# ccuchengwei/LongReadSelfCorrect

Hardware: NVIDIA B200
Metric: corrected Mbp/s (seed + FM-extend + DP/MSA fallback, default options) (higher is better)
Workload: dtype int64+f64

## Files before the change

include/pbsc.h:

```cpp
#ifndef PBSC_H
#define PBSC_H

#include <stddef.h>
#include <stdint.h>

#ifdef __cplusplus
extern "C" {
#endif

#define PBSC_OK 0
#define PBSC_ERR_ARG (-1)
#define PBSC_ERR_IO (-2)
#define PBSC_ERR_FORMAT (-3)
#define PBSC_ERR_CUDA (-4)
#define PBSC_ERR_LIMIT (-5)
#define PBSC_ERR_INTERNAL (-6)

#define PBSC_BWT 0
#define PBSC_RBWT 1

#define PBSC_WALK_OK 1
#define PBSC_WALK_HIGH_ERROR (-1)
#define PBSC_WALK_EXCEED_DEPTH (-2)
#define PBSC_WALK_EXCEED_LEAVES (-3)
// ... 110 lines not shown
int pbsc_batch_run(pbsc_batch* b, float* ms);
int pbsc_batch_result_size(pbsc_batch* b, uint64_t* piece_bytes, uint64_t* n_pieces);
int pbsc_batch_fetch(pbsc_batch* b, char* pieces_out, uint64_t pieces_cap, uint64_t* piece_offsets,
                     uint64_t piece_offsets_cap, uint64_t* first_piece, pbsc_read_stats* stats);
void pbsc_batch_destroy(pbsc_batch* b);

typedef struct pbsc_walk_log { int32_t src_start, trg_start, code, dp_failed; } pbsc_walk_log;
int pbsc_batch_debug_size(pbsc_batch* b, uint64_t* n_seeds, uint64_t* n_log);
int pbsc_batch_fetch_debug(pbsc_batch* b, pbsc_seed* seeds, uint64_t seeds_cap, uint64_t* seed_offsets, uint32_t* n_surviving, float* ratio,
                           uint64_t ratio_cap, pbsc_walk_log* log, uint64_t log_cap, uint64_t* log_offsets);

typedef struct pbsc_timing
{
    float h2d_ms, seed_ms, extend_ms, d2h_ms, total_ms;
    uint64_t kernel_launches;
    uint64_t seed_pairs;
    uint64_t rank_queries;
    float dp_ms;
    uint64_t dp_jobs;
    uint64_t dp_rows;
    float walk_ms;
    uint64_t walk_launches;
    uint64_t dp_thread_rows;
} pbsc_timing;
int pbsc_last_timing(pbsc_timing* t);
int pbsc_occ_counts(uint64_t* out, int reset);

#define PBSC_BUILD_NO_FORWARD 1
#define PBSC_BUILD_NO_REVERSE 2
int pbsc_build_index_files(const char* reads, const uint64_t* offsets, uint64_t n_reads, const char* prefix, int device, int flags);
int pbsc_build_bwt(const char* reads, const uint64_t* offsets, uint64_t n_reads, int reverse, int device, uint8_t** runs, uint64_t* n_runs,
                   uint64_t* n_symbols, uint32_t** lex_order);
void pbsc_free(void* p);

#ifdef __cplusplus
}
#endif
#endif
```

longreadselfcorrect_b200/api.py:

```python
from __future__ import annotations

import ctypes as C
import os
from dataclasses import dataclass

import numpy as np

_PKG = os.path.dirname(os.path.abspath(__file__))
LIB_PATH = os.environ.get("PBSC_LIB") or os.path.join(_PKG, "libpbsc.so")

PBSC_BWT, PBSC_RBWT = 0, 1


class PbscError(RuntimeError):
    def __init__(self, code: int, msg: str):
        super().__init__(f"pbsc error {code}: {msg}")
        self.code = code


class CParams(C.Structure):
    _fields_ = [
        ("pb_coverage", C.c_int32), ("error_rate", C.c_double), ("start_kmer", C.c_int32), ("next_target", C.c_int32),
        ("max_leaves", C.c_int32), ("idmer_len", C.c_int32), ("min_kmer", C.c_int32), ("genome", C.c_int32),
        ("mode", C.c_int32), ("manual", C.c_int32), ("adjust", C.c_int32), ("split", C.c_int32), ("no_dp", C.c_int32),
        ("offset", C.c_int32 * 3), ("pool", C.c_int32 * 8), ("n_pool", C.c_int32), ("scan_kmer", C.c_int32),
        ("kmer_up_bound", C.c_int32), ("radius", C.c_int32), ("hh_ratio", C.c_float),
        ("threshold", (C.c_float * 52) * 3), ("freqs_of_kmer", C.c_double * 101),
        ("debug_seed", C.c_int32), ("reserved", C.c_int32),
    ]


class CSeed(C.Structure):
    _fields_ = [("start", C.c_int32), ("len", C.c_int32), ("max_fixed_freq", C.c_int32), ("is_repeat", C.c_int32),
                ("start_best_k", C.c_int32), ("end_best_k", C.c_int32), ("hitchhiked", C.c_int32), ("static_k", C.c_int32)]


class CReadStats(C.Structure):
    _fields_ = [(n, C.c_int64) for n in ("total_reads_len", "corrected_len", "total_seed_num", "total_walk_num",
                                          "high_error_num", "exceed_depth_num", "exceed_leave_num", "fm_num", "dp_num",
                                          "seed_dis")] + [("merge", C.c_int32), ("n_pieces", C.c_int32)]


class CTiming(C.Structure):
    _fields_ = [("h2d_ms", C.c_float), ("seed_ms", C.c_float), ("extend_ms", C.c_float), ("d2h_ms", C.c_float),
                ("total_ms", C.c_float), ("kernel_launches", C.c_uint64), ("seed_pairs", C.c_uint64),
                ("rank_queries", C.c_uint64), ("dp_ms", C.c_float), ("dp_jobs", C.c_uint64), ("dp_rows", C.c_uint64),
                ("walk_ms", C.c_float), ("walk_launches", C.c_uint64), ("dp_thread_rows", C.c_uint64)]


SEED_DTYPE = np.dtype([("start", "<i4"), ("len", "<i4"), ("max_fixed_freq", "<i4"), ("is_repeat", "<i4"),
                       ("start_best_k", "<i4"), ("end_best_k", "<i4"), ("hitchhiked", "<i4"), ("static_k", "<i4")])
STATS_DTYPE = np.dtype([(n, "<i8") for n in ("total_reads_len", "corrected_len", "total_seed_num", "total_walk_num",
                                             "high_error_num", "exceed_depth_num", "exceed_leave_num", "fm_num",
                                             "dp_num", "seed_dis")] + [("merge", "<i4"), ("n_pieces", "<i4")])

WALK_LOG_DTYPE = np.dtype([("src_start", "<i4"), ("trg_start", "<i4"), ("code", "<i4"), ("dp_failed", "<i4")])

EXPORTED = ["pbsc_last_error", "pbsc_device_count", "pbsc_params_default", "pbsc_params_derive",
            "pbsc_threshold_table_text", "pbsc_index_create", "pbsc_index_load", "pbsc_index_create_synthetic",
            "pbsc_index_build_prefix_table", "pbsc_index_destroy", "pbsc_index_num_symbols", "pbsc_index_num_strings",
            "pbsc_index_device_bytes", "pbsc_index_get_symbols", "pbsc_findinterval_batch", "pbsc_findinterval_device",
            "pbsc_seed_batch", "pbsc_extend_batch", "pbsc_correct_batch", "pbsc_last_timing",
            "pbsc_batch_upload", "pbsc_batch_run", "pbsc_batch_result_size", "pbsc_batch_fetch", "pbsc_batch_destroy",
            "pbsc_host_alloc", "pbsc_host_free", "pbsc_trim", "pbsc_random_sector_bench",
            "pbsc_index_save", "pbsc_index_load_fmg", "pbsc_index_open", "pbsc_index_clone", "pbsc_index_blob_size",
            "pbsc_index_export_blob", "pbsc_index_import_blob", "pbsc_index_set_lanes", "pbsc_index_lanes",
            "pbsc_host_register", "pbsc_host_unregister", "pbsc_occ_counts",
            "pbsc_batch_debug_size", "pbsc_batch_fetch_debug",
            "pbsc_build_index_files", "pbsc_build_bwt", "pbsc_free"]

# ... 442 lines not shown
```

longreadselfcorrect_b200/csrc/pbsc_dp.cu:

```cuda
#include <cub/cub.cuh>
#include <stdio.h>
#include <stdlib.h>
#include <string.h>
#include <algorithm>
#include <vector>
#include <type_traits>
#include "pbsc_batch.cuh"
#include "pbsc_task.cuh"
#include <chrono>
#include "pbsc_dp.cuh"
#include "pbsc_dp_thread.cuh"
#include "pbsc_dp_msa.cuh"

namespace pbsc {

constexpr int DP_HALF = 100;
constexpr int DP_BW = 2 * DP_HALF + 1;
constexpr int DP_CPL = 7;
constexpr int DP_NEG = -(1 << 28);
constexpr int DP_WARPS = 8;

struct __align__(16) DpJob
{
    uint64_t lo[4];
// ... 579 lines not shown
__global__ void __launch_bounds__(128)
dp_job_keys_kernel(uint64_t j0, uint64_t j1, const DpJob* __restrict__ jobs, const DpRow* __restrict__ rows, uint64_t row_base, uint32_t* keys,
                   uint32_t* order)
{
    const uint64_t t = blockIdx.x * (uint64_t)blockDim.x + threadIdx.x;
    if (j0 + t >= j1) return;
    const DpJob J = jobs[j0 + t];
    const uint32_t nr = job_rows_of(J);
    const DpRow* R = rows + (J.row0 - row_base);
    uint32_t passing = 0, cost = 0;
    for (uint32_t r = 0; r < nr; r++)
    {
        const DpRow x = R[r];
        if (x.pass == 1) { passing++; cost += x.nops; }
    }
    if (passing < 3) cost = 0;
    keys[t] = 0xFFFFu - min(0xFFFFu, cost >> 3);
    order[t] = (uint32_t)t;
}

__global__ void __launch_bounds__(64)
dp_msa_kernel(uint64_t j0, uint64_t j1, const uint32_t* __restrict__ order, int deal, const DpJob* __restrict__ jobs, WalkTask* tasks,
              const DpRow* __restrict__ rows, uint64_t row_base, uint8_t* mem, uint64_t mem0, uint8_t* outpool, unsigned int* n_bad,
              uint32_t big_thr, uint32_t* big_list, unsigned int* n_big)
{
    const uint64_t tx = blockIdx.x * (uint64_t)blockDim.x + threadIdx.x;
    const uint64_t njc = j1 - j0;
    uint64_t rank = tx;
    if (order && deal)
    {
        const uint64_t n_warps = (njc + 31) / 32;
        rank = (tx & 31) * n_warps + (tx >> 5);
        if (tx >= n_warps * 32) return;
    }
    if (rank >= njc) return;
    const uint64_t jx = j0 + (order ? order[rank] : rank);
    const DpJob J = jobs[jx];
    WalkTask& tk = tasks[J.task];
    const uint32_t nr = job_rows_of(J);
    const DpRow* R = rows + (J.row0 - row_base);
    if (big_list)
    {
        uint32_t cost = 0, passing = 0;
        for (uint32_t r = 0; r < nr; r++) { const DpRow x = R[r]; if (x.pass == 1) { passing++; cost += x.nops; } }
        if (passing >= 3 && cost >= big_thr) { big_list[atomicAdd(n_big, 1u)] = (uint32_t)(jx - j0); return; }
    }
    JobView v;
    job_view(mem + (J.mem - mem0), J, nr, v);
    const MsaCtx ctx{tk, outpool};
    uint32_t n = 0;
    const int rc = msa::consensus(v, J.qlen, J.k, R, nr, ctx, n);
    if (rc == 1) { tk.dp_status = PBSC_DP_FEW_ROWS; return; }
    if (rc == 2) { atomicAdd(n_bad, 1u); tk.dp_status = PBSC_OVF_DP; return; }
    tk.out_len = n;
    tk.dp_status = PBSC_DP_OK;
}

constexpr int MSA_WARPS = 4;
__global__ void __launch_bounds__(MSA_WARPS * 32)
dp_msa_warp_kernel(uint64_t j0, const uint32_t* __restrict__ big_list, const unsigned int* __restrict__ n_big, unsigned long long* counter,
                   const DpJob* __restrict__ jobs, WalkTask* tasks, const DpRow* __restrict__ rows, uint64_t row_base, uint8_t* mem, uint64_t mem0,
                   uint8_t* outpool, unsigned int* n_bad)
{
    __shared__ unsigned int gap_counter[MSA_WARPS];
    const int lane = threadIdx.x & 31, warp = threadIdx.x >> 5;
    const unsigned long long n = *n_big;
    for (;;)
    {
        unsigned long long it = 0;
        if (lane == 0) it = atomicAdd(counter, 1ull);
        it = __shfl_sync(0xffffffffu, it, 0);
        if (it >= n) break;
        const uint64_t jx = j0 + big_list[it];
        const DpJob J = jobs[jx];
        WalkTask& tk = tasks[J.task];
        const uint32_t nr = job_rows_of(J);
        const DpRow* R = rows + (J.row0 - row_base);
        JobView v;
        job_view(mem + (J.mem - mem0), J, nr, v);
        const MsaCtx ctx{tk, outpool};
        uint32_t nout = 0;
        const int rc = msa::consensus_warp(v, J.qlen, J.k, R, nr, ctx, nout, &gap_counter[warp]);
        __syncwarp();
        if (lane == 0)
        {
            if (rc == 1) tk.dp_status = PBSC_DP_FEW_ROWS;
            else if (rc == 2) { atomicAdd(n_bad, 1u); tk.dp_status = PBSC_OVF_DP; }
            else { tk.out_len = nout; tk.dp_status = PBSC_DP_OK; }
        }
        __syncwarp();
    }
}

template <class T>
static cudaError_t arena(pbsc_index* idx, const char* name, size_t count, T** out) { return arena_get(idx, name, (count ? count : 1) * sizeof(T), (void**)out); }

DpStats& last_dp_stats() { static thread_local DpStats s; return s; }

struct DptPass
{
    bool on = false; uint64_t qmax = 0, arena_words = 0, min_rows = 0, read_words = 0; int blocks = 0;
    uint64_t flag_words() const { return on ? arena_words * (uint64_t)blocks : 0; }
};
template <class C>
static cudaError_t dpt_pass_setup(pbsc_index* idx, uint64_t q_longest, uint64_t q_prev_max, int cap_per_sm, DptPass& g)
{
    g.on = q_longest > q_prev_max;
    if (!g.on) return cudaSuccess;
    g.qmax = std::min<uint64_t>((uint64_t)C::QMAX, q_longest);
    g.arena_words = 32ull * g.qmax * dpt::WMAX;
    cudaError_t e = cudaFuncSetAttribute(dp_align_thread_kernel<C>, cudaFuncAttributeMaxDynamicSharedMemorySize, C::SMEM);
    if (e != cudaSuccess) return e;
    int per = 0;
    e = cudaOccupancyMaxActiveBlocksPerMultiprocessor(&per, dp_align_thread_kernel<C>, C::NT, C::SMEM);
// ... 18 lines not shown
}

int run_dp_fallback(pbsc_index* idx, const pbsc_params* p, DeviceBatch& b, void* tasks_v, uint64_t n_items, const uint32_t* list, uint8_t* outpool,
                    uint32_t q_cap, uint64_t* launches)
{
    WalkTask* tasks = (WalkTask*)tasks_v;
    cudaStream_t st = idx->stream;
    if (n_items == 0) return PBSC_OK;
    const bool htrace = getenv("PBSC_ROUND_TRACE") != nullptr;
    auto h0 = std::chrono::steady_clock::now();
    auto hmark = [&](const char* what) {
        if (!htrace) return;
        const auto now = std::chrono::steady_clock::now();
        const double ms = std::chrono::duration<double, std::milli>(now - h0).count();
        if (ms > 2.0) fprintf(stderr, "[pbsc round trace]     dp host: %-22s %8.2f ms\n", what, ms);
        h0 = now;
    };
    DpJob* jobs; uint64_t *job_rows, *job_bytes, *row_off, *mem_off; unsigned int* cnt; unsigned long long* qctr;
    PBSC_CUDA(arena(idx, "dp.jobs", n_items, &jobs));
    PBSC_CUDA(arena(idx, "dp.job_rows", n_items + 1, &job_rows));
    PBSC_CUDA(arena(idx, "dp.job_bytes", n_items + 1, &job_bytes));
    PBSC_CUDA(arena(idx, "dp.row_off", n_items + 1, &row_off));
    PBSC_CUDA(arena(idx, "dp.mem_off", n_items + 1, &mem_off));
    PBSC_CUDA(arena(idx, "dp.cnt", 4, &cnt));
    PBSC_CUDA(arena(idx, "dp.qctr", 4, &qctr));
    PBSC_CUDA(cudaMemsetAsync(cnt, 0, 16, st));
    cudaEvent_t ev[2];
    PBSC_CUDA(cudaEventCreate(&ev[0])); PBSC_CUDA(cudaEventCreate(&ev[1]));
    struct EvGuard { cudaEvent_t* e; ~EvGuard() { cudaEventDestroy(e[0]); cudaEventDestroy(e[1]); } } guard{ev};
    PBSC_CUDA(cudaEventRecord(ev[0], st));
    dp_collect_kernel<<<(unsigned)((n_items + 127) / 128), 128, 0, st>>>(idx->dev, n_items, list, tasks, b.codes.p, b.offsets.p, (uint32_t)p->pb_coverage,
                                                                        jobs, job_rows, job_bytes, cnt);
    unsigned int hcnt[4] = {0, 0, 0, 0};
    PBSC_CUDA(cudaMemcpyAsync(hcnt, cnt, 16, cudaMemcpyDeviceToHost, st));
    PBSC_CUDA(cudaStreamSynchronize(st));
    if (launches) *launches += 1;
    const uint64_t nj = hcnt[0];
    DpStats& S = last_dp_stats();
    hmark("collect + sync");
    if (nj == 0) return PBSC_OK;
    {
        size_t tb = 0, tb2 = 0;
        cub::DeviceScan::ExclusiveSum(nullptr, tb, job_rows, row_off, (int)(nj + 1), st);
        cub::DeviceScan::ExclusiveSum(nullptr, tb2, job_bytes, mem_off, (int)(nj + 1), st);
        tb = std::max(tb, tb2);
        uint8_t* tmp;
        PBSC_CUDA(arena(idx, "dp.cubtmp", tb, &tmp));
        PBSC_CUDA(cudaMemsetAsync(job_rows + nj, 0, 8, st));
        PBSC_CUDA(cudaMemsetAsync(job_bytes + nj, 0, 8, st));
        cub::DeviceScan::ExclusiveSum(tmp, tb, job_rows, row_off, (int)(nj + 1), st);
        cub::DeviceScan::ExclusiveSum(tmp, tb, job_bytes, mem_off, (int)(nj + 1), st);
        dp_offsets_kernel<<<(unsigned)((nj + 255) / 256), 256, 0, st>>>(nj, jobs, row_off, mem_off);
    }
    std::vector<uint64_t> h_row(nj + 1), h_mem(nj + 1);
    PBSC_CUDA(cudaMemcpyAsync(h_row.data(), row_off, (nj + 1) * 8, cudaMemcpyDeviceToHost, st));
    PBSC_CUDA(cudaMemcpyAsync(h_mem.data(), mem_off, (nj + 1) * 8, cudaMemcpyDeviceToHost, st));
// ... 65 lines not shown
        cub::DeviceRadixSort::SortPairs(nullptr, sort_bytes, tkeys, tkeys2, torder, torder2, (int)max_rows, 0, DPT_KEY_BITS, st);
        PBSC_CUDA(arena(idx, "dp.sorttmp", sort_bytes, &sort_tmp));
        PBSC_CUDA(arena(idx, "dp.tflags", std::max(pass_s.flag_words(), std::max(pass_l.flag_words(), pass_h.flag_words())), &tslabs));
        PBSC_CUDA(arena(idx, "dp.treads", std::max<uint64_t>(1, std::max(pass_l.on ? pass_l.read_words : 0, pass_h.on ? pass_h.read_words : 0)), &treads));
    }
    int sort_jobs = 0;
    if (const char* e = getenv("PBSC_DP_SORT_JOBS")) sort_jobs = atoi(e);
    uint32_t *jkeys = nullptr, *jkeys2 = nullptr, *jord = nullptr, *jord2 = nullptr;
    uint8_t* jsort_tmp = nullptr;
    size_t jsort_bytes = 0;
    if (sort_jobs)
    {
        PBSC_CUDA(arena(idx, "dp.jkeys", nj, &jkeys));
        PBSC_CUDA(arena(idx, "dp.jkeys2", nj, &jkeys2));
        PBSC_CUDA(arena(idx, "dp.jord", nj, &jord));
        PBSC_CUDA(arena(idx, "dp.jord2", nj, &jord2));
        cub::DeviceRadixSort::SortPairs(nullptr, jsort_bytes, jkeys, jkeys2, jord, jord2, (int)nj, 0, 16, st);
        PBSC_CUDA(arena(idx, "dp.jsorttmp", jsort_bytes, &jsort_tmp));
    }
    uint32_t msa_big_thr = 8192;
    if (const char* e = getenv("PBSC_MSA_WARP_MIN")) msa_big_thr = atoll(e) < 0 ? 0xffffffffu : (uint32_t)atoll(e);
    uint32_t* msa_big = nullptr;
    unsigned long long* msa_q = nullptr;
    PBSC_CUDA(arena(idx, "dp.msa_big", nj, &msa_big));
    PBSC_CUDA(arena(idx, "dp.msa_q", 2, &msa_q));
    struct Prof
    {
        bool on = false; cudaStream_t st; std::vector<std::pair<const char*, cudaEvent_t>> ev;
        void mark(const char* name) { if (!on) return; cudaEvent_t e; cudaEventCreate(&e); cudaEventRecord(e, st); ev.emplace_back(name, e); }
        void report()
        {
            if (!on || ev.size() < 2) return;
            cudaEventSynchronize(ev.back().second);
            std::vector<std::pair<const char*, float>> acc;
            for (size_t x = 1; x < ev.size(); x++)
            {
                float ms = 0; cudaEventElapsedTime(&ms, ev[x - 1].second, ev[x].second);
                bool found = false;
                for (auto& a : acc) if (!strcmp(a.first, ev[x].first)) { a.second += ms; found = true; }
                if (!found) acc.emplace_back(ev[x].first, ms);
            }
            fprintf(stderr, "[pbsc dp profile]");
            for (auto& a : acc) fprintf(stderr, " %s %.1f ms;", a.first, a.second);
            fprintf(stderr, "\n");
            for (auto& e : ev) cudaEventDestroy(e.second);
        }
    } prof;
    prof.st = st;
    if (const char* e = getenv("PBSC_DP_PROFILE")) prof.on = atoi(e) != 0;
    hmark("pass setup + arenas");
    prof.mark("start");
    for (uint64_t j0 = 0; j0 < nj;)
    {
        uint64_t j1 = j0 + 1;
        while (j1 < nj && h_mem[j1 + 1] - h_mem[j0] <= pool_bytes) j1++;
        const uint64_t nrows = h_row[j1] - h_row[j0], njc = j1 - j0;
        dp_rows_kernel<<<(unsigned)((njc + 127) / 128), 128, 0, st>>>(j0, j1, jobs, tasks, b.codes.p, b.offsets.p, mem, h_mem[j0], rows, h_row[j0]);
        dp_retrieve_kernel<<<(unsigned)((nrows + 127) / 128), 128, 0, st>>>(idx->dev, nrows, rows, jobs, mem, h_mem[j0]);
        prof.mark("rows+retrieve");
        PBSC_CUDA(cudaMemsetAsync(qctr, 0, 32, st));
        if (pass_s.on)
        {
            dpt_pass_launch<DptShort>(pass_s, st, nrows, rows, jobs, tasks, mem, h_mem[j0], tkeys, tkeys2, torder, torder2, sort_tmp, sort_bytes, tslabs,
                                      qctr + 1, cnt, treads);
            prof.mark("align_thread_256");
            if (launches) *launches += 4;
        }
        if (pass_l.on)
        {
            dpt_pass_launch<DptLong>(pass_l, st, nrows, rows, jobs, tasks, mem, h_mem[j0], tkeys, tkeys2, torder, torder2, sort_tmp, sort_bytes, tslabs,
                                     qctr + 1, cnt, treads);
            prof.mark("align_thread_1024");
            if (launches) *launches += 4;
        }
        if (pass_h.on)
        {
            dpt_pass_launch<DptHuge>(pass_h, st, nrows, rows, jobs, tasks, mem, h_mem[j0], tkeys, tkeys2, torder, torder2, sort_tmp, sort_bytes, tslabs,
                                     qctr + 1, cnt, treads);
            prof.mark("align_thread_4000");
            if (launches) *launches += 4;
        }
        const int nb = (int)std::min<uint64_t>((uint64_t)ablocks, (nrows + DP_WARPS * 32 - 1) / (DP_WARPS * 32));
        dp_align_kernel<<<nb, DP_WARPS * 32, 0, st>>>(nrows, rows, jobs, tasks, mem, h_mem[j0], slabs, arena_words, qctr, cnt + 1);
        prof.mark("align_warp");
        const uint32_t* jorder = nullptr;
        if (sort_jobs)
        {
            dp_job_keys_kernel<<<(unsigned)((njc + 127) / 128), 128, 0, st>>>(j0, j1, jobs, rows, h_row[j0], jkeys, jord);
            size_t sb = jsort_bytes;
            cub::DeviceRadixSort::SortPairs(jsort_tmp, sb, jkeys, jkeys2, jord, jord2, (int)njc, 0, 16, st);
            jorder = jord2;
            if (launches) *launches += 3;
        }
        PBSC_CUDA(cudaMemsetAsync(msa_q, 0, 16, st));
        dp_msa_kernel<<<(unsigned)((((njc + 31) / 32) * 32 + 63) / 64), 64, 0, st>>>(j0, j1, jorder, sort_jobs == 1, jobs, tasks, rows, h_row[j0], mem,
                                                                                         h_mem[j0], outpool, cnt + 1, msa_big_thr,
                                                                                         msa_big_thr != 0xffffffffu ? msa_big : nullptr, (unsigned int*)(msa_q + 1));
        prof.mark("msa");
        if (msa_big_thr != 0xffffffffu)
        {
            const int wb = (int)std::min<uint64_t>((uint64_t)idx->sm_count * 4, (njc + MSA_WARPS - 1) / MSA_WARPS);
            dp_msa_warp_kernel<<<wb, MSA_WARPS * 32, 0, st>>>(j0, msa_big, (const unsigned int*)(msa_q + 1), msa_q, jobs, tasks, rows, h_row[j0], mem, h_mem[j0],
                                                              outpool, cnt + 1);
            prof.mark("msa_warp");
            if (launches) *launches += 1;
        }
        PBSC_CUDA(cudaGetLastError());
        if (launches) *launches += 4;
        S.chunks++;
        j0 = j1;
    }
    PBSC_CUDA(cudaEventRecord(ev[1], st));
    hmark("chunk loop (launches)");
    prof.report();
    PBSC_CUDA(cudaMemcpyAsync(hcnt, cnt, 12, cudaMemcpyDeviceToHost, st));
    PBSC_CUDA(cudaStreamSynchronize(st));
    S.bad += hcnt[1];
    S.thread_rows += hcnt[2];
    PBSC_OCC_TAKE(3, st);
    float ms = 0;
    cudaEventElapsedTime(&ms, ev[0], ev[1]);
    S.ms += ms;
    return PBSC_OK;
}

}
```

longreadselfcorrect_b200/csrc/pbsc_dp.cuh:

```cuda
#ifndef PBSC_DP_CUH
#define PBSC_DP_CUH

#include "pbsc_batch.cuh"

namespace pbsc {

struct DpStats { uint64_t jobs = 0, rows = 0, chunks = 0, bad = 0, thread_rows = 0; float ms = 0; };
DpStats& last_dp_stats();

int run_dp_fallback(pbsc_index* idx, const pbsc_params* p, DeviceBatch& b, void* tasks, uint64_t n_items, const uint32_t* list, uint8_t* outpool,
                    uint32_t q_cap, uint64_t* launches);

}
#endif
```

longreadselfcorrect_b200/csrc/pbsc_dp_msa.cuh:

```cuda
#ifndef PBSC_DP_MSA_CUH
#define PBSC_DP_MSA_CUH

#include <stdint.h>

#if defined(__CUDACC__)
#define PBSC_MSA_HD __host__ __device__ __forceinline__
#define PBSC_MSA_ALIGN(n) __align__(n)
#else
#define PBSC_MSA_HD inline
#define PBSC_MSA_ALIGN(n) alignas(n)
#endif

namespace pbsc {

constexpr int OP_M = 0, OP_I = 1, OP_D = 2;

struct PBSC_MSA_ALIGN(16) DpRow
{
    uint32_t job, local;
    uint32_t len, seq_start;
    uint32_t nops;
    int32_t start0, start1;
    uint32_t pass;
};
// ... 94 lines not shown
#endif
        for (int s = 0; s < 5; s++) if ((int)cnt[s] > maxCount) { maxSym = s; maxCount = cnt[s]; }
        const int baseCount = cnt[baseSym];
        return (maxCount >= baseCount && baseCount < minCall) ? maxSym : baseSym;
    };
    bool over = false;
    for (uint32_t p = 0; p < qlen && !over; p++)
    {
        if (p >= 1)
            for (uint32_t g = v.head[p]; g; g = v.pool[g - 1].next)
            {
                const int s = call(v.pool[g - 1].cnt, 4);
                if (s != 4) { if (n >= cap) { over = true; break; } out[n++] = (uint8_t)s; }
            }
        if (over) break;
        const int s = call(v.baseCnt + p * 5, (int)q[p]);
        if (s != 4) { if (n >= cap) { over = true; break; } out[n++] = (uint8_t)s; }
    }
    if (over || n < k) return 2;
    n_out = n;
    return 0;
}

#if defined(__CUDACC__)
template <class Ctx>
__device__ __forceinline__ int consensus_warp(const JobView& v, const uint32_t qlen, const uint32_t k, const DpRow* R, const uint32_t nr, const Ctx& ctx,
                                              uint32_t& n_out, unsigned int* gap_counter)
{
    const unsigned FULLW = 0xffffffffu;
    const int lane = threadIdx.x & 31;
    uint32_t passing = 0;
    for (uint32_t r = lane; r < nr; r += 32) passing += R[r].pass == 1;
    #pragma unroll
    for (int o = 16; o > 0; o >>= 1) passing += __shfl_xor_sync(FULLW, passing, o);
    if (passing < 3) return 1;
    const uint8_t* q = v.q;
    for (uint32_t p = lane; p <= qlen; p += 32)
    {
        #pragma unroll
        for (int c = 0; c < 5; c++) v.baseCnt[p * 5 + c] = 0;
        v.startAt[p] = p == 0 ? 1 : 0; v.head[p] = 0; v.tail[p] = 0;
        if (p < qlen) v.baseCnt[p * 5 + q[p]] = 1;
    }
    if (lane == 0) *gap_counter = 0;
    __syncwarp();
    const uint32_t gapCap = dp_gap_cap(qlen);
    bool bad = false;
    for (uint32_t r = 0; r < nr; r++)
    {
        if (R[r].pass != 1) continue;
        const uint8_t* buf = v.rows + (uint64_t)R[r].local * v.rowBytes;
        const uint8_t* s2 = buf + R[r].seq_start;
        const uint8_t* ops = buf + v.seqBytes;
        const int nops = (int)R[r].nops;
        const int chunk = (nops + 31) / 32;
        int t0 = min(lane * chunk, nops);
        while (t0 > 0 && t0 < nops && ops[nops - t0] == OP_I) t0++;
        int t1 = __shfl_down_sync(FULLW, t0, 1);
        if (lane == 31) t1 = nops;
        uint32_t md = 0, mi = 0;
        for (int t = t0; t < t1; t++) { const int op = ops[nops - 1 - t]; md += op != OP_I; mi += op != OP_D; }
        uint32_t pmd = md, pmi = mi;
        #pragma unroll
        for (int o = 1; o < 32; o <<= 1)
        {
            const uint32_t a = __shfl_up_sync(FULLW, pmd, o), b = __shfl_up_sync(FULLW, pmi, o);
            if (lane >= o) { pmd += a; pmi += b; }
        }
        uint32_t p = (uint32_t)R[r].start0 + (pmd - md), inc = (uint32_t)R[r].start1 + (pmi - mi);
        bool firstOp = t0 == 0;
        uint32_t cur = (t0 == 0 || t0 >= t1) ? 0 : v.head[p];
        int t = t0;
        while (t < t1)
        {
            const int op = ops[nops - 1 - t];
            if (cur)
            {
                GapCol& g = v.pool[cur - 1];
                if (op == OP_I) { g.cnt[s2[inc]]++; inc++; t++; firstOp = false; }
                else g.cnt[4]++;
                cur = g.next;
            }
            else if (op == OP_I)
            {
                const uint32_t slot = atomicAdd(gap_counter, 1u);
                if (slot >= gapCap) { bad = true; break; }
                uint32_t cover = 0;
                #pragma unroll
                for (int s = 0; s < 5; s++) cover += v.baseCnt[p * 5 + s];
                GapCol g;
                g.cnt[0] = g.cnt[1] = g.cnt[2] = g.cnt[3] = 0; g.pad = 0; g.next = 0;
                g.cnt[4] = (uint16_t)(cover - v.startAt[p]);
                g.cnt[s2[inc]] = 1;
                v.pool[slot] = g;
                if (v.tail[p]) v.pool[v.tail[p] - 1].next = slot + 1; else v.head[p] = slot + 1;
                v.tail[p] = slot + 1;
                inc++; t++; firstOp = false;
            }
            else
            {
                if (p >= qlen) { bad = true; break; }
                v.baseCnt[p * 5 + (op == OP_M ? s2[inc] : 4)]++;
                if (op == OP_M) inc++;
                if (firstOp) v.startAt[p]++;
                firstOp = false;
                p++; t++;
                cur = v.head[p];
            }
        }
        __syncwarp();
        if (__any_sync(FULLW, bad)) return 2;
    }
    const int minCall = ctx.min_call();
    uint8_t* out = ctx.out();
    const uint32_t cap = ctx.cap();
    auto call = [&](const uint16_t* cnt, int baseSym) -> int
    {
        int maxSym = -1, maxCount = -1;
        #pragma unroll
        for (int s = 0; s < 5; s++) if ((int)cnt[s] > maxCount) { maxSym = s; maxCount = cnt[s]; }
        const int baseCount = cnt[baseSym];
        return (maxCount >= baseCount && baseCount < minCall) ? maxSym : baseSym;
    };
    const uint32_t blk = (qlen + 31) / 32;
    const uint32_t pa = min((uint32_t)lane * blk, qlen), pb = min(pa + blk, qlen);
    uint32_t n = 0;
    #pragma unroll 1
    for (int pass = 0; pass < 2; pass++)
    {
        uint32_t w = 0;
        if (pass == 1)
        {
            uint32_t incl = n;
            #pragma unroll
            for (int o = 1; o < 32; o <<= 1) { const uint32_t a = __shfl_up_sync(FULLW, incl, o); if (lane >= o) incl += a; }
            const uint32_t total = __shfl_sync(FULLW, incl, 31);
            if (total > cap || total < k) return 2;
            n_out = total;
            w = incl - n;
        }
        for (uint32_t p = pa; p < pb; p++)
        {
            if (p >= 1)
                for (uint32_t g = v.head[p]; g; g = v.pool[g - 1].next)
                {
                    const int s = call(v.pool[g - 1].cnt, 4);
                    if (s != 4) { if (pass == 0) n++; else out[w++] = (uint8_t)s; }
                }
            const int s = call(v.baseCnt + p * 5, (int)q[p]);
            if (s != 4) { if (pass == 0) n++; else out[w++] = (uint8_t)s; }
        }
    }
    return 0;
}
#endif

}
}

#endif
```

longreadselfcorrect_b200/csrc/pbsc_index.cu:

```cuda
#include <math.h>
#include <string.h>
#include <sys/stat.h>
#include <algorithm>
#include <cub/cub.cuh>
#include <mutex>
#include <map>
#include <fstream>
#include <sstream>
#include "pbsc_internal.h"

namespace pbsc {

static thread_local std::string g_err;
void set_error(const char* fmt, ...)
{
    char buf[1024];
    va_list ap;
    va_start(ap, fmt);
    vsnprintf(buf, sizeof buf, fmt, ap);
    va_end(ap);
    g_err = buf;
}
int cuda_fail(cudaError_t e, const char* what, const char* file, int line)
{
// ... 978 lines not shown
}
PBSC_CATCH_ALL("pbsc_threshold_table_text")

int pbsc_occ_counts(uint64_t* out, int reset)
{
    if (!out) return PBSC_ERR_ARG;
    unsigned long long* c = occ_counts();
    for (int i = 0; i < 5; i++) { out[i] = c[i]; if (reset) c[i] = 0; }
#ifdef PBSC_COUNT_OCC
    return 1;
#else
    return 0;
#endif
}

int pbsc_last_timing(pbsc_timing* t)
{
    if (!t) return PBSC_ERR_ARG;
    const Timing& s = last_timing();
    t->h2d_ms = s.h2d_ms; t->seed_ms = s.seed_ms; t->extend_ms = s.extend_ms; t->d2h_ms = s.d2h_ms; t->total_ms = s.total_ms;
    t->kernel_launches = s.kernel_launches; t->seed_pairs = s.seed_pairs; t->rank_queries = s.rank_queries;
    t->dp_ms = s.dp_ms; t->dp_jobs = s.dp_jobs; t->dp_rows = s.dp_rows;
    t->walk_ms = s.walk_ms; t->walk_launches = s.walk_launches; t->dp_thread_rows = s.dp_thread_rows;
    return PBSC_OK;
}

}
```

longreadselfcorrect_b200/csrc/pbsc_internal.h:

```cpp
#ifndef PBSC_INTERNAL_H
#define PBSC_INTERNAL_H

#include <cuda_runtime.h>
#include <stdarg.h>
#include <stdint.h>
#include <stdio.h>
#include <stdlib.h>
#include <chrono>
#include <exception>
#include <map>
#include <new>
#include <mutex>
#include <condition_variable>
#include <string>
#include <vector>
#include "../../include/pbsc.h"
#include "fm_table.cuh"
#include "pbsc_status.h"

struct pbsc_index
{
    int device = 0;
    pbsc::FmIndexDev dev;
    pbsc::FmBlock* d_blocks[2] = {nullptr, nullptr};
// ... 70 lines not shown
        const auto t0 = std::chrono::steady_clock::now();
        if (a.p) cudaFree(a.p);
        a.p = nullptr; a.cap = 0;
        const size_t want = bytes + bytes / 8 + 256;
        cudaError_t e = cudaMalloc(&a.p, want);
        if (e != cudaSuccess) return e;
        a.cap = want;
        if (tr) fprintf(stderr, "[pbsc round trace]     arena %-16s -> %8.1f MB in %7.2f ms\n", name, want / 1048576.0,
                        std::chrono::duration<double, std::milli>(std::chrono::steady_clock::now() - t0).count());
    }
    *out = a.p;
    return cudaSuccess;
}

struct Timing
{
    float h2d_ms = 0, seed_ms = 0, extend_ms = 0, d2h_ms = 0, total_ms = 0;
    uint64_t kernel_launches = 0, seed_pairs = 0, rank_queries = 0;
    float dp_ms = 0;
    uint64_t dp_jobs = 0, dp_rows = 0;
    float walk_ms = 0;
    uint64_t walk_launches = 0;
    uint64_t dp_thread_rows = 0;
};
Timing& last_timing();

#define PBSC_MAX_LANES 4
int lane_acquire(pbsc_index* primary, int idmer_len, pbsc_index** lane);
void lane_release(pbsc_index* primary, pbsc_index* lane);
int ensure_idmer_table(pbsc_index* idx, int idmer_len);

inline int base_code(char b) { switch (b) { case 'A': return 0; case 'C': return 1; case 'G': return 2; case 'T': return 3; default: return -1; } }

}
#endif
```

longreadselfcorrect_b200/csrc/pbsc_pipeline.cu:

```cuda
#include <string.h>
#include <stdlib.h>
#include <chrono>
#include <memory>
#include <new>
#include "pbsc_batch.cuh"
#include "pbsc_dp.cuh"

using namespace pbsc;

struct pbsc_batch
{
    pbsc_index* idx = nullptr;
    pbsc_params params;
    DeviceBatch b;
    SeedBuffers s;
    Workspace w;
    std::vector<uint64_t> h_offsets;
    std::vector<uint64_t> h_packed_off;
    std::vector<uint32_t> h_bounds;
    std::vector<pbsc_read_stats> h_stats;
    bool ran = false, fetched = false;
    float h2d_ms = 0, seed_ms = 0, extend_ms = 0, d2h_ms = 0;
    uint64_t launches = 0, walks = 0;
    cudaStream_t cs = nullptr;
// ... 147 lines not shown
        if (ovf_pool) bt->w.pool_nodes *= 4;
        if (ovf_pieces || ovf_other)
        {
            rc = alloc_extend_workspace(idx, &bt->params, bt->h_offsets, bt->b, bt->s, bt->w, st);
            if (rc != PBSC_OK) break;
        }
    }
    if (rc == PBSC_OK)
    {
        cudaEventElapsedTime(&bt->seed_ms, e[0], e[1]);
        bt->extend_ms = extend_total;
        unsigned long long hw = 0;
        cudaMemcpy(&hw, bt->w.counters.p + 1, 8, cudaMemcpyDeviceToHost);
        bt->walks = hw;
        bt->ran = true;
        bt->fetched = false;
        if (ms) *ms = bt->seed_ms + bt->extend_ms;
        Timing& T = last_timing();
        T.h2d_ms = bt->h2d_ms; T.seed_ms = bt->seed_ms; T.extend_ms = bt->extend_ms; T.d2h_ms = 0;
        T.total_ms = bt->h2d_ms + bt->seed_ms + bt->extend_ms;
        T.kernel_launches = bt->launches; T.seed_pairs = bt->walks;
        const DpStats& D = last_dp_stats();
        T.dp_ms = D.ms; T.dp_jobs = D.jobs; T.dp_rows = D.rows; T.dp_thread_rows = D.thread_rows;
        if (D.bad) { set_error("DP fallback: %llu alignments or consensus buffers outside this build's limits", (unsigned long long)D.bad); rc = PBSC_ERR_LIMIT; }
        if (grew && rc == PBSC_OK)
        {
            std::lock_guard<std::mutex> lk(primary->run_mu);
            primary->learned_node_cap = std::max(primary->learned_node_cap, bt->w.node_cap);
            primary->learned_piece_factor = std::max(primary->learned_piece_factor, bt->w.piece_factor);
            primary->learned_pool_nodes = std::max(primary->learned_pool_nodes, bt->w.pool_nodes);
        }
    }
    return rc;
}

extern "C" {

int pbsc_batch_upload(pbsc_index* idx, const pbsc_params* p, const char* reads, const uint64_t* offsets, uint64_t n_reads, pbsc_batch** out)
{
    if (!idx || !p || !reads || !offsets || !out) { set_error("pbsc_batch_upload: null argument"); return PBSC_ERR_ARG; }
    *out = nullptr;
    return guarded("pbsc_batch_upload", [&] { return batch_upload_impl(idx, p, reads, offsets, n_reads, out); });
}

int pbsc_batch_run(pbsc_batch* bt, float* ms)
{
// ... 222 lines not shown
```

Baseline: 82.25.

## Keep MSA consensus column counts in shared memory for warp-level jobs

After: 80.48 (median of 6 runs). 2.1% lower.

```diff
diff --git a/include/pbsc.h b/include/pbsc.h
--- a/include/pbsc.h
+++ b/include/pbsc.h
@@ -156,6 +156,7 @@
     float walk_ms;
     uint64_t walk_launches;
     uint64_t dp_thread_rows;
+    uint64_t dp_msa_shared_jobs;
 } pbsc_timing;
 int pbsc_last_timing(pbsc_timing* t);
 int pbsc_occ_counts(uint64_t* out, int reset);
diff --git a/longreadselfcorrect_b200/api.py b/longreadselfcorrect_b200/api.py
--- a/longreadselfcorrect_b200/api.py
+++ b/longreadselfcorrect_b200/api.py
@@ -45,7 +45,8 @@
     _fields_ = [("h2d_ms", C.c_float), ("seed_ms", C.c_float), ("extend_ms", C.c_float), ("d2h_ms", C.c_float),
                 ("total_ms", C.c_float), ("kernel_launches", C.c_uint64), ("seed_pairs", C.c_uint64),
                 ("rank_queries", C.c_uint64), ("dp_ms", C.c_float), ("dp_jobs", C.c_uint64), ("dp_rows", C.c_uint64),
-                ("walk_ms", C.c_float), ("walk_launches", C.c_uint64), ("dp_thread_rows", C.c_uint64)]
+                ("walk_ms", C.c_float), ("walk_launches", C.c_uint64), ("dp_thread_rows", C.c_uint64),
+                ("dp_msa_shared_jobs", C.c_uint64)]
 
 
 SEED_DTYPE = np.dtype([("start", "<i4"), ("len", "<i4"), ("max_fixed_freq", "<i4"), ("is_repeat", "<i4"),
diff --git a/longreadselfcorrect_b200/csrc/pbsc_dp.cu b/longreadselfcorrect_b200/csrc/pbsc_dp.cu
--- a/longreadselfcorrect_b200/csrc/pbsc_dp.cu
+++ b/longreadselfcorrect_b200/csrc/pbsc_dp.cu
@@ -625,7 +625,7 @@
 __global__ void __launch_bounds__(64)
 dp_msa_kernel(uint64_t j0, uint64_t j1, const uint32_t* __restrict__ order, int deal, const DpJob* __restrict__ jobs, WalkTask* tasks,
               const DpRow* __restrict__ rows, uint64_t row_base, uint8_t* mem, uint64_t mem0, uint8_t* outpool, unsigned int* n_bad,
-              uint32_t big_thr, uint32_t* big_list, unsigned int* n_big)
+              uint32_t big_thr, uint32_t* big_list, unsigned int* n_big, uint32_t long_q)
 {
     const uint64_t tx = blockIdx.x * (uint64_t)blockDim.x + threadIdx.x;
     const uint64_t njc = j1 - j0;
@@ -646,7 +646,12 @@
     {
         uint32_t cost = 0, passing = 0;
         for (uint32_t r = 0; r < nr; r++) { const DpRow x = R[r]; if (x.pass == 1) { passing++; cost += x.nops; } }
-        if (passing >= 3 && cost >= big_thr) { big_list[atomicAdd(n_big, 1u)] = (uint32_t)(jx - j0); return; }
+        if (passing >= 3 && cost >= big_thr)
+        {
+            const int b = J.qlen > long_q;
+            big_list[b * njc + atomicAdd(n_big + b, 1u)] = (uint32_t)(jx - j0);
+            return;
+        }
     }
     JobView v;
     job_view(mem + (J.mem - mem0), J, nr, v);
@@ -660,14 +665,23 @@
 }
 
 constexpr int MSA_WARPS = 4;
-__global__ void __launch_bounds__(MSA_WARPS * 32)
+__host__ __device__ inline uint32_t msa_warp_bytes(uint32_t slice_q)
+{
+    return msa::shared_cols_bytes(slice_q) + (uint32_t)dp_row_bytes(slice_q, dp_max_len(slice_q));
+}
+__global__ void __launch_bounds__(MSA_WARPS * 32, 1)
 dp_msa_warp_kernel(uint64_t j0, const uint32_t* __restrict__ big_list, const unsigned int* __restrict__ n_big, unsigned long long* counter,
                    const DpJob* __restrict__ jobs, WalkTask* tasks, const DpRow* __restrict__ rows, uint64_t row_base, uint8_t* mem, uint64_t mem0,
-                   uint8_t* outpool, unsigned int* n_bad)
-{
+                   uint8_t* outpool, unsigned int* n_bad, uint32_t slice_q, unsigned int* n_shared)
+{
+    extern __shared__ __align__(16) uint8_t msa_smem[];
     __shared__ unsigned int gap_counter[MSA_WARPS];
     const int lane = threadIdx.x & 31, warp = threadIdx.x >> 5;
+    uint8_t* slice = msa_smem + (size_t)warp * msa_warp_bytes(slice_q);
+    const msa::SharedCols sc = msa::shared_cols(slice, slice_q);
+    uint8_t* stage = slice + msa::shared_cols_bytes(slice_q);
     const unsigned long long n = *n_big;
+    unsigned int shared_jobs = 0;
     for (;;)
     {
         unsigned long long it = 0;
@@ -683,7 +697,9 @@
         job_view(mem + (J.mem - mem0), J, nr, v);
         const MsaCtx ctx{tk, outpool};
         uint32_t nout = 0;
-        const int rc = msa::consensus_warp(v, J.qlen, J.k, R, nr, ctx, nout, &gap_counter[warp]);
+        int rc;
+        if (J.qlen <= slice_q) { rc = msa::consensus_warp(v, sc, J.qlen, J.k, R, nr, ctx, nout, &gap_counter[warp], stage); shared_jobs++; }
+        else rc = msa::consensus_warp(v, msa::global_cols(v), J.qlen, J.k, R, nr, ctx, nout, &gap_counter[warp], (uint8_t*)nullptr);
         __syncwarp();
         if (lane == 0)
         {
@@ -693,6 +709,37 @@
         }
         __syncwarp();
     }
+    if (lane == 0 && shared_jobs) atomicAdd(n_shared, shared_jobs);
+}
+
+constexpr uint32_t MSA_SHORT_Q = 480, MSA_LONG_Q = 2048;
+struct MsaPass
+{
+    uint32_t slice_q = 0; int warps = MSA_WARPS, blocks = 0; size_t smem = 0;
+};
+static cudaError_t msa_pass_setup(pbsc_index* idx, uint32_t slice_q, bool verbose, MsaPass& g)
+{
+    g.slice_q = slice_q;
+    g.warps = MSA_WARPS;
+    g.smem = 0;
+    if (slice_q == 0) { g.blocks = idx->sm_count * 4; return cudaSuccess; }
+    int optin = 0;
+    cudaError_t e = cudaDeviceGetAttribute(&optin, cudaDevAttrMaxSharedMemoryPerBlockOptin, idx->device);
+    if (e != cudaSuccess) return e;
+    auto block_bytes = [&](uint32_t q) { const size_t slice = msa_warp_bytes(q); return std::min<size_t>(MSA_WARPS, (size_t)optin / slice) * slice; };
+    const size_t slice = msa_warp_bytes(slice_q);
+    g.warps = (int)(block_bytes(slice_q) / slice);
+    if (g.warps < 1) return cudaErrorInvalidValue;
+    g.smem = (size_t)g.warps * slice;
+    e = cudaFuncSetAttribute(dp_msa_warp_kernel, cudaFuncAttributeMaxDynamicSharedMemorySize, (int)std::max(g.smem, block_bytes(MSA_LONG_Q)));
+    if (e != cudaSuccess) return e;
+    int per = 0;
+    e = cudaOccupancyMaxActiveBlocksPerMultiprocessor(&per, dp_msa_warp_kernel, g.warps * 32, g.smem);
+    if (e != cudaSuccess) return e;
+    g.blocks = idx->sm_count * std::max(per, 1);
+    if (verbose)
+        fprintf(stderr, "[pbsc msa] slice for %u bases: %zu B, %d warps x %d blocks per SM\n", slice_q, slice, g.warps, per);
+    return cudaSuccess;
 }
 
 template <class T>
@@ -757,16 +804,16 @@
     PBSC_CUDA(arena(idx, "dp.job_bytes", n_items + 1, &job_bytes));
     PBSC_CUDA(arena(idx, "dp.row_off", n_items + 1, &row_off));
     PBSC_CUDA(arena(idx, "dp.mem_off", n_items + 1, &mem_off));
-    PBSC_CUDA(arena(idx, "dp.cnt", 4, &cnt));
+    PBSC_CUDA(arena(idx, "dp.cnt", 5, &cnt));
     PBSC_CUDA(arena(idx, "dp.qctr", 4, &qctr));
-    PBSC_CUDA(cudaMemsetAsync(cnt, 0, 16, st));
+    PBSC_CUDA(cudaMemsetAsync(cnt, 0, 20, st));
     cudaEvent_t ev[2];
     PBSC_CUDA(cudaEventCreate(&ev[0])); PBSC_CUDA(cudaEventCreate(&ev[1]));
     struct EvGuard { cudaEvent_t* e; ~EvGuard() { cudaEventDestroy(e[0]); cudaEventDestroy(e[1]); } } guard{ev};
     PBSC_CUDA(cudaEventRecord(ev[0], st));
     dp_collect_kernel<<<(unsigned)((n_items + 127) / 128), 128, 0, st>>>(idx->dev, n_items, list, tasks, b.codes.p, b.offsets.p, (uint32_t)p->pb_coverage,
                                                                         jobs, job_rows, job_bytes, cnt);
-    unsigned int hcnt[4] = {0, 0, 0, 0};
+    unsigned int hcnt[5] = {0, 0, 0, 0, 0};
     PBSC_CUDA(cudaMemcpyAsync(hcnt, cnt, 16, cudaMemcpyDeviceToHost, st));
     PBSC_CUDA(cudaStreamSynchronize(st));
     if (launches) *launches += 1;
@@ -878,8 +925,18 @@
     if (const char* e = getenv("PBSC_MSA_WARP_MIN")) msa_big_thr = atoll(e) < 0 ? 0xffffffffu : (uint32_t)atoll(e);
     uint32_t* msa_big = nullptr;
     unsigned long long* msa_q = nullptr;
-    PBSC_CUDA(arena(idx, "dp.msa_big", nj, &msa_big));
-    PBSC_CUDA(arena(idx, "dp.msa_q", 2, &msa_q));
+    PBSC_CUDA(arena(idx, "dp.msa_big", 2 * nj, &msa_big));
+    PBSC_CUDA(arena(idx, "dp.msa_q", 3, &msa_q));
+    bool msa_shared = true;
+    if (const char* e = getenv("PBSC_MSA_SHARED")) msa_shared = atoi(e) != 0;
+    const bool dp_profile = getenv("PBSC_DP_PROFILE") && atoi(getenv("PBSC_DP_PROFILE")) != 0;
+    MsaPass msa_s, msa_l;
+    const bool msa_two = msa_shared && q_longest > MSA_SHORT_Q;
+    if (msa_big_thr != 0xffffffffu)
+    {
+        PBSC_CUDA(msa_pass_setup(idx, msa_shared ? (uint32_t)std::min<uint64_t>(MSA_SHORT_Q, q_longest) : 0, dp_profile, msa_s));
+        if (msa_two) PBSC_CUDA(msa_pass_setup(idx, (uint32_t)std::min<uint64_t>(MSA_LONG_Q, q_longest), dp_profile, msa_l));
+    }
     struct Prof
     {
         bool on = false; cudaStream_t st; std::vector<std::pair<const char*, cudaEvent_t>> ev;
@@ -903,7 +960,7 @@
         }
     } prof;
     prof.st = st;
-    if (const char* e = getenv("PBSC_DP_PROFILE")) prof.on = atoi(e) != 0;
+    prof.on = dp_profile;
     hmark("pass setup + arenas");
     prof.mark("start");
     for (uint64_t j0 = 0; j0 < nj;)
@@ -948,18 +1005,23 @@
             jorder = jord2;
             if (launches) *launches += 3;
         }
-        PBSC_CUDA(cudaMemsetAsync(msa_q, 0, 16, st));
+        PBSC_CUDA(cudaMemsetAsync(msa_q, 0, 24, st));
         dp_msa_kernel<<<(unsigned)((((njc + 31) / 32) * 32 + 63) / 64), 64, 0, st>>>(j0, j1, jorder, sort_jobs == 1, jobs, tasks, rows, h_row[j0], mem,
                                                                                          h_mem[j0], outpool, cnt + 1, msa_big_thr,
-                                                                                         msa_big_thr != 0xffffffffu ? msa_big : nullptr, (unsigned int*)(msa_q + 1));
+                                                                                         msa_big_thr != 0xffffffffu ? msa_big : nullptr, (unsigned int*)(msa_q + 2),
+                                                                                         msa_two ? MSA_SHORT_Q : 0xffffffffu);
         prof.mark("msa");
         if (msa_big_thr != 0xffffffffu)
         {
-            const int wb = (int)std::min<uint64_t>((uint64_t)idx->sm_count * 4, (njc + MSA_WARPS - 1) / MSA_WARPS);
-            dp_msa_warp_kernel<<<wb, MSA_WARPS * 32, 0, st>>>(j0, msa_big, (const unsigned int*)(msa_q + 1), msa_q, jobs, tasks, rows, h_row[j0], mem, h_mem[j0],
-                                                              outpool, cnt + 1);
-            prof.mark("msa_warp");
-            if (launches) *launches += 1;
+            for (int b = 0; b < (msa_two ? 2 : 1); b++)
+            {
+                const MsaPass& g = b ? msa_l : msa_s;
+                const int wb = (int)std::min<uint64_t>((uint64_t)g.blocks, (njc + g.warps - 1) / g.warps);
+                dp_msa_warp_kernel<<<wb, g.warps * 32, g.smem, st>>>(j0, msa_big + b * njc, (const unsigned int*)(msa_q + 2) + b, msa_q + b, jobs, tasks, rows,
+                                                                     h_row[j0], mem, h_mem[j0], outpool, cnt + 1, g.slice_q, cnt + 4);
+                prof.mark(b ? "msa_warp_long" : "msa_warp");
+                if (launches) *launches += 1;
+            }
         }
         PBSC_CUDA(cudaGetLastError());
         if (launches) *launches += 4;
@@ -969,10 +1031,11 @@
     PBSC_CUDA(cudaEventRecord(ev[1], st));
     hmark("chunk loop (launches)");
     prof.report();
-    PBSC_CUDA(cudaMemcpyAsync(hcnt, cnt, 12, cudaMemcpyDeviceToHost, st));
+    PBSC_CUDA(cudaMemcpyAsync(hcnt, cnt, 20, cudaMemcpyDeviceToHost, st));
     PBSC_CUDA(cudaStreamSynchronize(st));
     S.bad += hcnt[1];
     S.thread_rows += hcnt[2];
+    S.msa_shared_jobs += hcnt[4];
     PBSC_OCC_TAKE(3, st);
     float ms = 0;
     cudaEventElapsedTime(&ms, ev[0], ev[1]);
diff --git a/longreadselfcorrect_b200/csrc/pbsc_dp.cuh b/longreadselfcorrect_b200/csrc/pbsc_dp.cuh
--- a/longreadselfcorrect_b200/csrc/pbsc_dp.cuh
+++ b/longreadselfcorrect_b200/csrc/pbsc_dp.cuh
@@ -5,7 +5,7 @@
 
 namespace pbsc {
 
-struct DpStats { uint64_t jobs = 0, rows = 0, chunks = 0, bad = 0, thread_rows = 0; float ms = 0; };
+struct DpStats { uint64_t jobs = 0, rows = 0, chunks = 0, bad = 0, thread_rows = 0, msa_shared_jobs = 0; float ms = 0; };
 DpStats& last_dp_stats();
 
 int run_dp_fallback(pbsc_index* idx, const pbsc_params* p, DeviceBatch& b, void* tasks, uint64_t n_items, const uint32_t* list, uint8_t* outpool,
diff --git a/longreadselfcorrect_b200/csrc/pbsc_dp_msa.cuh b/longreadselfcorrect_b200/csrc/pbsc_dp_msa.cuh
--- a/longreadselfcorrect_b200/csrc/pbsc_dp_msa.cuh
+++ b/longreadselfcorrect_b200/csrc/pbsc_dp_msa.cuh
@@ -140,10 +140,131 @@
     return 0;
 }
 
+struct PBSC_MSA_ALIGN(4) GapCol16 { uint16_t cnt[5]; uint16_t next; };
+template <class Idx, class Gap>
+struct ColStore { uint16_t* baseCnt; uint16_t* startAt; Idx* head; Idx* tail; Gap* pool; };
+using GlobalCols = ColStore<uint32_t, GapCol>;
+using SharedCols = ColStore<uint16_t, GapCol16>;
+PBSC_MSA_HD GlobalCols global_cols(const JobView& v) { return GlobalCols{v.baseCnt, v.startAt, v.head, v.tail, v.pool}; }
+
+constexpr uint32_t SHARED_QMAX = 21000;
+static_assert(3 * SHARED_QMAX + 128 < 65536, "SharedCols links are 16 bits");
+PBSC_MSA_HD uint32_t msa_align16(uint32_t x) { return (x + 15u) & ~15u; }
+PBSC_MSA_HD uint32_t shared_cols_bytes(uint32_t qmax)
+{
+    const uint32_t np = qmax + 1;
+    return msa_align16(np * 10) + 3 * msa_align16(np * 2) + msa_align16(dp_gap_cap(qmax) * (uint32_t)sizeof(GapCol16));
+}
+PBSC_MSA_HD SharedCols shared_cols(uint8_t* slice, uint32_t qmax)
+{
+    const uint32_t np = qmax + 1;
+    SharedCols s;
+    s.baseCnt = (uint16_t*)slice; slice += msa_align16(np * 10);
+    s.startAt = (uint16_t*)slice; slice += msa_align16(np * 2);
+    s.head = (uint16_t*)slice; slice += msa_align16(np * 2);
+    s.tail = (uint16_t*)slice; slice += msa_align16(np * 2);
+    s.pool = (GapCol16*)slice;
+    return s;
+}
+
+template <class S>
+PBSC_MSA_HD void init_column(const S& s, const uint8_t* q, uint32_t qlen, uint32_t p)
+{
+    for (int c = 0; c < 5; c++) s.baseCnt[p * 5 + c] = 0;
+    s.startAt[p] = p == 0 ? 1 : 0; s.head[p] = 0; s.tail[p] = 0;
+    if (p < qlen) s.baseCnt[p * 5 + q[p]] = 1;
+}
+
+PBSC_MSA_HD int segment_start(const uint8_t* ops, int nops, int lane)
+{
+    const int chunk = (nops + 31) / 32;
+    int t0 = lane * chunk < nops ? lane * chunk : nops;
+    while (t0 > 0 && t0 < nops && ops[nops - t0] == OP_I) t0++;
+    return t0;
+}
+
+PBSC_MSA_HD void segment_moves(const uint8_t* ops, int nops, int t0, int t1, uint32_t& md, uint32_t& mi)
+{
+    md = 0; mi = 0;
+    for (int t = t0; t < t1; t++) { const int op = ops[nops - 1 - t]; md += op != OP_I; mi += op != OP_D; }
+}
+
+template <class Idx, class Gap, class NewGap>
+PBSC_MSA_HD bool add_segment(const ColStore<Idx, Gap>& s, const uint8_t* ops, const uint8_t* s2, int nops, int t0, int t1, uint32_t p, uint32_t inc,
+                             uint32_t qlen, NewGap&& new_gap)
+{
+    const uint32_t gapCap = dp_gap_cap(qlen);
+    bool firstOp = t0 == 0;
+    uint32_t cur = (t0 == 0 || t0 >= t1) ? 0 : s.head[p];
+    int t = t0;
+    while (t < t1)
+    {
+        const int op = ops[nops - 1 - t];
+        if (cur)
+        {
+            Gap& g = s.pool[cur - 1];
+            if (op == OP_I) { g.cnt[s2[inc]]++; inc++; t++; firstOp = false; }
+            else g.cnt[4]++;
+            cur = g.next;
+        }
+        else if (op == OP_I)
+        {
+            const uint32_t slot = new_gap();
+            if (slot >= gapCap) return false;
+            uint32_t cover = 0;
+            for (int c = 0; c < 5; c++) cover += s.baseCnt[p * 5 + c];
+            const int sym = s2[inc];
+            Gap g;
+            for (int c = 0; c < 5; c++) g.cnt[c] = sym == c ? 1 : c == 4 ? (uint16_t)(cover - s.startAt[p]) : 0;
+            g.next = 0;
+            s.pool[slot] = g;
+            if (s.tail[p]) s.pool[s.tail[p] - 1].next = slot + 1; else s.head[p] = slot + 1;
+            s.tail[p] = slot + 1;
+            inc++; t++; firstOp = false;
+        }
+        else
+        {
+            if (p >= qlen) return false;
+            s.baseCnt[p * 5 + (op == OP_M ? s2[inc] : 4)]++;
+            if (op == OP_M) inc++;
+            if (firstOp) s.startAt[p]++;
+            firstOp = false;
+            p++; t++;
+            cur = s.head[p];
+        }
+    }
+    return true;
+}
+
+template <class S>
+PBSC_MSA_HD uint32_t call_range(const S& s, const uint8_t* q, uint32_t pa, uint32_t pb, int minCall, uint8_t* out)
+{
+    auto call = [&](const uint16_t* cnt, int baseSym) -> int
+    {
+        int maxSym = -1, maxCount = -1;
+        for (int c = 0; c < 5; c++) if ((int)cnt[c] > maxCount) { maxSym = c; maxCount = cnt[c]; }
+        const int baseCount = cnt[baseSym];
+        return (maxCount >= baseCount && baseCount < minCall) ? maxSym : baseSym;
+    };
+    uint32_t n = 0;
+    for (uint32_t p = pa; p < pb; p++)
+    {
+        if (p >= 1)
+            for (uint32_t g = s.head[p]; g; g = s.pool[g - 1].next)
+            {
+                const int c = call(s.pool[g - 1].cnt, 4);
+                if (c != 4) { if (out) out[n] = (uint8_t)c; n++; }
+            }
+        const int c = call(s.baseCnt + p * 5, (int)q[p]);
+        if (c != 4) { if (out) out[n] = (uint8_t)c; n++; }
+    }
+    return n;
+}
+
 #if defined(__CUDACC__)
-template <class Ctx>
-__device__ __forceinline__ int consensus_warp(const JobView& v, const uint32_t qlen, const uint32_t k, const DpRow* R, const uint32_t nr, const Ctx& ctx,
-                                              uint32_t& n_out, unsigned int* gap_counter)
+template <class S, class Ctx>
+__device__ __forceinline__ int consensus_warp(const JobView& v, const S& s, const uint32_t qlen, const uint32_t k, const DpRow* R, const uint32_t nr,
+                                              const Ctx& ctx, uint32_t& n_out, unsigned int* gap_counter, uint8_t* stage)
 {
     const unsigned FULLW = 0xffffffffu;
     const int lane = threadIdx.x & 31;
@@ -153,31 +274,30 @@
     for (int o = 16; o > 0; o >>= 1) passing += __shfl_xor_sync(FULLW, passing, o);
     if (passing < 3) return 1;
     const uint8_t* q = v.q;
-    for (uint32_t p = lane; p <= qlen; p += 32)
-    {
-        #pragma unroll
-        for (int c = 0; c < 5; c++) v.baseCnt[p * 5 + c] = 0;
-        v.startAt[p] = p == 0 ? 1 : 0; v.head[p] = 0; v.tail[p] = 0;
-        if (p < qlen) v.baseCnt[p * 5 + q[p]] = 1;
-    }
+    for (uint32_t p = lane; p <= qlen; p += 32) init_column(s, q, qlen, p);
     if (lane == 0) *gap_counter = 0;
     __syncwarp();
-    const uint32_t gapCap = dp_gap_cap(qlen);
-    bool bad = false;
     for (uint32_t r = 0; r < nr; r++)
     {
-        if (R[r].pass != 1) continue;
-        const uint8_t* buf = v.rows + (uint64_t)R[r].local * v.rowBytes;
-        const uint8_t* s2 = buf + R[r].seq_start;
+        const DpRow row = R[r];
+        if (row.pass != 1) continue;
+        const uint8_t* buf = v.rows + (uint64_t)row.local * v.rowBytes;
+        const int nops = (int)row.nops;
+        if (stage)
+        {
+            const uint32_t lo = row.seq_start & ~15u, hi = (uint32_t)v.seqBytes + (((uint32_t)nops + 15u) & ~15u);
+            __syncwarp();
+            for (uint32_t x = lo + 16u * lane; x < hi; x += 512u) *(uint4*)(stage + x) = *(const uint4*)(buf + x);
+            __syncwarp();
+            buf = stage;
+        }
+        const uint8_t* s2 = buf + row.seq_start;
         const uint8_t* ops = buf + v.seqBytes;
-        const int nops = (int)R[r].nops;
-        const int chunk = (nops + 31) / 32;
-        int t0 = min(lane * chunk, nops);
-        while (t0 > 0 && t0 < nops && ops[nops - t0] == OP_I) t0++;
+        const int t0 = segment_start(ops, nops, lane);
         int t1 = __shfl_down_sync(FULLW, t0, 1);
         if (lane == 31) t1 = nops;
-        uint32_t md = 0, mi = 0;
-        for (int t = t0; t < t1; t++) { const int op = ops[nops - 1 - t]; md += op != OP_I; mi += op != OP_D; }
+        uint32_t md, mi;
+        segment_moves(ops, nops, t0, t1, md, mi);
         uint32_t pmd = md, pmi = mi;
         #pragma unroll
         for (int o = 1; o < 32; o <<= 1)
@@ -185,90 +305,22 @@
             const uint32_t a = __shfl_up_sync(FULLW, pmd, o), b = __shfl_up_sync(FULLW, pmi, o);
             if (lane >= o) { pmd += a; pmi += b; }
         }
-        uint32_t p = (uint32_t)R[r].start0 + (pmd - md), inc = (uint32_t)R[r].start1 + (pmi - mi);
-        bool firstOp = t0 == 0;
-        uint32_t cur = (t0 == 0 || t0 >= t1) ? 0 : v.head[p];
-        int t = t0;
-        while (t < t1)
-        {
-            const int op = ops[nops - 1 - t];
-            if (cur)
-            {
-                GapCol& g = v.pool[cur - 1];
-                if (op == OP_I) { g.cnt[s2[inc]]++; inc++; t++; firstOp = false; }
-                else g.cnt[4]++;
-                cur = g.next;
-            }
-            else if (op == OP_I)
-            {
-                const uint32_t slot = atomicAdd(gap_counter, 1u);
-                if (slot >= gapCap) { bad = true; break; }
-                uint32_t cover = 0;
-                #pragma unroll
-                for (int s = 0; s < 5; s++) cover += v.baseCnt[p * 5 + s];
-                GapCol g;
-                g.cnt[0] = g.cnt[1] = g.cnt[2] = g.cnt[3] = 0; g.pad = 0; g.next = 0;
-                g.cnt[4] = (uint16_t)(cover - v.startAt[p]);
-                g.cnt[s2[inc]] = 1;
-                v.pool[slot] = g;
-                if (v.tail[p]) v.pool[v.tail[p] - 1].next = slot + 1; else v.head[p] = slot + 1;
-                v.tail[p] = slot + 1;
-                inc++; t++; firstOp = false;
-            }
-            else
-            {
-                if (p >= qlen) { bad = true; break; }
-                v.baseCnt[p * 5 + (op == OP_M ? s2[inc] : 4)]++;
-                if (op == OP_M) inc++;
-                if (firstOp) v.startAt[p]++;
-                firstOp = false;
-                p++; t++;
-                cur = v.head[p];
-            }
-        }
+        const bool ok = add_segment(s, ops, s2, nops, t0, t1, (uint32_t)row.start0 + (pmd - md), (uint32_t)row.start1 + (pmi - mi), qlen,
+                                    [&]() { return atomicAdd(gap_counter, 1u); });
         __syncwarp();
-        if (__any_sync(FULLW, bad)) return 2;
-    }
-    const int minCall = ctx.min_call();
-    uint8_t* out = ctx.out();
-    const uint32_t cap = ctx.cap();
-    auto call = [&](const uint16_t* cnt, int baseSym) -> int
-    {
-        int maxSym = -1, maxCount = -1;
-        #pragma unroll
-        for (int s = 0; s < 5; s++) if ((int)cnt[s] > maxCount) { maxSym = s; maxCount = cnt[s]; }
-        const int baseCount = cnt[baseSym];
-        return (maxCount >= baseCount && baseCount < minCall) ? maxSym : baseSym;
-    };
+        if (__any_sync(FULLW, !ok)) return 2;
+    }
     const uint32_t blk = (qlen + 31) / 32;
     const uint32_t pa = min((uint32_t)lane * blk, qlen), pb = min(pa + blk, qlen);
-    uint32_t n = 0;
-    #pragma unroll 1
-    for (int pass = 0; pass < 2; pass++)
-    {
-        uint32_t w = 0;
-        if (pass == 1)
-        {
-            uint32_t incl = n;
-            #pragma unroll
-            for (int o = 1; o < 32; o <<= 1) { const uint32_t a = __shfl_up_sync(FULLW, incl, o); if (lane >= o) incl += a; }
-            const uint32_t total = __shfl_sync(FULLW, incl, 31);
-            if (total > cap || total < k) return 2;
-            n_out = total;
-            w = incl - n;
-        }
-        for (uint32_t p = pa; p < pb; p++)
-        {
-            if (p >= 1)
-                for (uint32_t g = v.head[p]; g; g = v.pool[g - 1].next)
-                {
-                    const int s = call(v.pool[g - 1].cnt, 4);
-                    if (s != 4) { if (pass == 0) n++; else out[w++] = (uint8_t)s; }
-                }
-            const int s = call(v.baseCnt + p * 5, (int)q[p]);
-            if (s != 4) { if (pass == 0) n++; else out[w++] = (uint8_t)s; }
-        }
-    }
+    const int minCall = ctx.min_call();
+    const uint32_t n = call_range(s, q, pa, pb, minCall, nullptr);
+    uint32_t incl = n;
+    #pragma unroll
+    for (int o = 1; o < 32; o <<= 1) { const uint32_t a = __shfl_up_sync(FULLW, incl, o); if (lane >= o) incl += a; }
+    const uint32_t total = __shfl_sync(FULLW, incl, 31);
+    if (total > ctx.cap() || total < k) return 2;
+    n_out = total;
+    call_range(s, q, pa, pb, minCall, ctx.out() + (incl - n));
     return 0;
 }
 #endif
diff --git a/longreadselfcorrect_b200/csrc/pbsc_index.cu b/longreadselfcorrect_b200/csrc/pbsc_index.cu
--- a/longreadselfcorrect_b200/csrc/pbsc_index.cu
+++ b/longreadselfcorrect_b200/csrc/pbsc_index.cu
@@ -1024,7 +1024,8 @@
     t->kernel_launches = s.kernel_launches; t->seed_pairs = s.seed_pairs; t->rank_queries = s.rank_queries;
     t->dp_ms = s.dp_ms; t->dp_jobs = s.dp_jobs; t->dp_rows = s.dp_rows;
     t->walk_ms = s.walk_ms; t->walk_launches = s.walk_launches; t->dp_thread_rows = s.dp_thread_rows;
-    return PBSC_OK;
-}
-
-}
+    t->dp_msa_shared_jobs = s.dp_msa_shared_jobs;
+    return PBSC_OK;
+}
+
+}
diff --git a/longreadselfcorrect_b200/csrc/pbsc_internal.h b/longreadselfcorrect_b200/csrc/pbsc_internal.h
--- a/longreadselfcorrect_b200/csrc/pbsc_internal.h
+++ b/longreadselfcorrect_b200/csrc/pbsc_internal.h
@@ -116,6 +116,7 @@
     float walk_ms = 0;
     uint64_t walk_launches = 0;
     uint64_t dp_thread_rows = 0;
+    uint64_t dp_msa_shared_jobs = 0;
 };
 Timing& last_timing();
 
diff --git a/longreadselfcorrect_b200/csrc/pbsc_pipeline.cu b/longreadselfcorrect_b200/csrc/pbsc_pipeline.cu
--- a/longreadselfcorrect_b200/csrc/pbsc_pipeline.cu
+++ b/longreadselfcorrect_b200/csrc/pbsc_pipeline.cu
@@ -193,6 +193,7 @@
         T.kernel_launches = bt->launches; T.seed_pairs = bt->walks;
         const DpStats& D = last_dp_stats();
         T.dp_ms = D.ms; T.dp_jobs = D.jobs; T.dp_rows = D.rows; T.dp_thread_rows = D.thread_rows;
+        T.dp_msa_shared_jobs = D.msa_shared_jobs;
         if (D.bad) { set_error("DP fallback: %llu alignments or consensus buffers outside this build's limits", (unsigned long long)D.bad); rc = PBSC_ERR_LIMIT; }
         if (grew && rc == PBSC_OK)
         {
```
